# interactiveaudiolab/ppgs

Hardware: AMD Instinct MI355X
Metric: PPG frames/sec (whole node), mel repr, batch=32x1000 frames (higher is better)
Workload: dtype bf16; 1 GPU; configs[1]: mel representation, batch=32 x 1000 frames per GPU, audio resident in HBM -> (32,40,1000) fp32 posteriors in HBM; batch=32, frames=1000, per_gpu_batches=1, parallelism=utterance-sharded x1, no data-path collective

## Files before the change

ppgs_amd/csrc/ppg_frontend.hip:

```cpp
#include "ppg_lds.h"
#include "ppg_launch.h"

#include <hip/hip_fp16.h>

namespace {

constexpr int NFFT = 1024;
constexpr int HOP = 160;
constexpr int NBINS = 513;
constexpr int NMELS = 80;
constexpr int PADR = (NFFT - HOP) / 2;
constexpr int FPB = ppg::kFrontendFrames;
constexpr int SEG = NFFT + (FPB - 1) * HOP;
constexpr int BUF = NFFT + NFFT / 16;
constexpr int MSEG = ppg::kMelSegment;
constexpr int NS = ppg::kMelSteps;
constexpr int MROW = 1088;
__device__ __forceinline__ int sigma(int c) { return (0x6c >> (2 * c)) & 3; }

constexpr int OFF_TW = 0;
constexpr int SEGP = (SEG + 255) / 256 * 256;
constexpr int OFF_SEG = OFF_TW + 64 * 8;
constexpr int OFF_FFT = OFF_SEG + 2 * SEGP * 4;
constexpr int OFF_MAG = OFF_FFT + 4 * BUF * 8;
constexpr int LDS_BYTES = OFF_MAG + FPB * MROW;
constexpr int TEAMS = 2;
constexpr int CU_LDS_BYTES = 163840;
static_assert(2 * LDS_BYTES <= CU_LDS_BYTES && LDS_BYTES % 16 == 0, "two teams per CU; a two-team workgroup = the CU's LDS");
static_assert(OFF_MAG % 16 == 0 && MROW % 16 == 0, "fragment reads are 16-byte aligned");

typedef float cplx __attribute__((ext_vector_type(2)));
__device__ __forceinline__ cplx cadd(cplx a, cplx b) { return a + b; }
__device__ __forceinline__ cplx csub(cplx a, cplx b) { return a - b; }
__device__ __forceinline__ cplx cadd_mi(cplx a, cplx b) {
    cplx r;
    asm("v_pk_add_f32 %0, %1, %2 op_sel:[1,0] op_sel_hi:[0,1] neg_hi:[1,0]" : "=v"(r) : "v"(b), "v"(a));
    return r;
}
__device__ __forceinline__ cplx csub_mi(cplx a, cplx b) {
    cplx r;
    asm("v_pk_add_f32 %0, %1, %2 op_sel:[1,0] op_sel_hi:[0,1] neg_lo:[1,0]" : "=v"(r) : "v"(b), "v"(a));
    return r;
}
__device__ __forceinline__ cplx cmul(cplx a, cplx w) {
    cplx t, r;
    asm("v_pk_mul_f32 %0, %1, %2 op_sel:[0,0] op_sel_hi:[0,1]" : "=v"(t) : "v"(a), "v"(w));
    asm("v_fma_f32 %0, -%1, %2, %3" : "=v"(r.x) : "v"(a.y), "v"(w.y), "v"(t.x));
    asm("v_fma_f32 %0, %1, %2, %3" : "=v"(r.y) : "v"(a.y), "v"(w.x), "v"(t.y));
    return r;
}

template <bool CMI = false>
__device__ __forceinline__ void radix4(cplx& A, cplx& B, cplx& C, cplx& D) {
    const cplx apc = CMI ? cadd_mi(A, C) : cadd(A, C), amc = CMI ? csub_mi(A, C) : csub(A, C);
    const cplx bpd = cadd(B, D), bmd = csub(B, D);
    A = cadd(apc, bpd);
    B = cadd_mi(amc, bmd);
    C = csub(apc, bpd);
    D = csub_mi(amc, bmd);
}

template <int M>
__device__ __forceinline__ cplx w16() {
    constexpr float c1 = 0.92387953251128674f, s1 = 0.38268343236508977f, r = 0.70710678118654752f;
    if constexpr (M == 1) return cplx{c1, -s1};
    else if constexpr (M == 2) return cplx{r, -r};
    else if constexpr (M == 3) return cplx{s1, -c1};
    else if constexpr (M == 6) return cplx{-r, -r};
    else { static_assert(M == 9, "exponent"); return cplx{-c1, s1}; }
}

__device__ __forceinline__ void dft16(cplx (&x)[16]) {
#pragma unroll
    for (int r = 0; r < 4; ++r) radix4(x[r], x[r + 4], x[r + 8], x[r + 12]);
    x[5] = cmul(x[5], w16<1>());  x[9] = cmul(x[9], w16<2>());   x[13] = cmul(x[13], w16<3>());
    x[6] = cmul(x[6], w16<2>());   x[14] = cmul(x[14], w16<6>());
    x[7] = cmul(x[7], w16<3>());  x[11] = cmul(x[11], w16<6>()); x[15] = cmul(x[15], w16<9>());
    radix4(x[0], x[1], x[2], x[3]);
    radix4(x[4], x[5], x[6], x[7]);
    radix4<true>(x[8], x[9], x[10], x[11]);
    radix4(x[12], x[13], x[14], x[15]);
    cplx t;
#define PPG_SWAP(a, b) t = x[a]; x[a] = x[b]; x[b] = t;
    PPG_SWAP(1, 4) PPG_SWAP(2, 8) PPG_SWAP(3, 12) PPG_SWAP(6, 9) PPG_SWAP(7, 13) PPG_SWAP(11, 14)
#undef PPG_SWAP
}

__device__ __forceinline__ int pad(int i) { return i + (i >> 4); }

__device__ __forceinline__ void wave_sync() {
    asm volatile("s_waitcnt lgkmcnt(0)" ::: "memory");
    __builtin_amdgcn_fence(__ATOMIC_ACQ_REL, "wavefront");
    __builtin_amdgcn_wave_barrier();
}

template <bool SPEC, class SRC>
__device__ __forceinline__ void frontend_body(
    const ppg::FrontendTables& tb, const SRC& src, int total_groups, int wide_ok, __half* __restrict__ spec, __half* __restrict__ mel)
{
    extern __shared__ __attribute__((aligned(16))) char smem_all[];
    const int team = TEAMS == 1 ? 0 : __builtin_amdgcn_readfirstlane((int)(threadIdx.x >> 8));
    char* smem = smem_all + team * LDS_BYTES;
    cplx* tw = reinterpret_cast<cplx*>(smem + OFF_TW);
    float* seg0 = reinterpret_cast<float*>(smem + OFF_SEG);

    const int tid = threadIdx.x & 255;
    const int lane = tid & 63;
    const int wave = __builtin_amdgcn_readfirstlane(tid >> 6);
    cplx* buf = reinterpret_cast<cplx*>(smem + OFF_FFT) + wave * BUF;

    if (tid < 64) { const float2 w = tb.twiddle[16 * tid]; tw[tid] = cplx{w.x, w.y}; }
    reinterpret_cast<uint32_t*>(smem + OFF_MAG + (tid >> 4) * MROW + 1024)[tid & 15] = 0u;

    float hreg[16];
    cplx t1[16];
#pragma unroll
    for (int j = 0; j < 16; ++j) hreg[j] = tb.hann[lane + 64 * j];
#pragma unroll
    for (int k = 1; k < 16; ++k) { const float2 w = tb.twiddle[lane * k]; t1[k] = cplx{w.x, w.y}; }

    int step_frag[NS], step_off[NS], step_block[NS];
#pragma unroll
    for (int i = 0; i < NS; ++i) {
        const int4 e = tb.mel_prog[wave * NS + i];
        step_frag[i] = __builtin_amdgcn_readfirstlane(e.x);
        step_off[i] = __builtin_amdgcn_readfirstlane(e.y);
        step_block[i] = __builtin_amdgcn_readfirstlane(e.z);
    }

    auto stage = [&](int grp, int into) { src.stage(tb, grp, into, seg0, wave, lane, wide_ok); };
    const int stride = TEAMS * gridDim.x;
    const int first_group = TEAMS * blockIdx.x + team;
    if (first_group < total_groups) stage(first_group, 0);
    asm volatile("s_waitcnt vmcnt(0)" ::: "memory");

#ifdef PPG_FE_TIMING
    int stamp_group = 0;
    auto stamp = [&](int k) {
        if (tb.dbg && blockIdx.x == 0 && lane == 0 && stamp_group == 2) tb.dbg[wave * 16 + k] = __builtin_amdgcn_s_memtime();
    };
#else
    auto stamp = [&](int) {};
#endif
    int half = 0;
    const int trips = (total_groups - TEAMS * (int)blockIdx.x + stride - 1) / stride;
    int grp = first_group;
    for (int trip = 0; trip < trips; ++trip, grp += stride, half ^= 1) {
        const bool active = grp < total_groups;
        int b, f0, frames;
        src.group(grp, active, b, f0, frames);
        const float* seg = seg0 + half * SEGP;
        int pitch = src.pitch(frames);
        asm volatile("" : "+s"(pitch));
#ifdef PPG_FE_TIMING
        ++stamp_group;
#endif
        stamp(0);
        __syncthreads();
        stamp(1);

        auto transform = [&](const int j, const bool verify = false) {
            const int fa = f0 + 2 * j;
            if (fa >= frames) return;
            cplx x[16];
            {
                const float* sa = seg + (2 * j) * HOP + lane;
#pragma unroll
                for (int i = 0; i < 16; ++i) {
                    x[i] = cplx{sa[64 * i], sa[64 * i + HOP]} * hreg[i];
                }
                dft16(x);
#pragma unroll
                for (int k = 1; k < 16; ++k) x[k] = cmul(x[k], t1[k]);
#pragma unroll
                for (int k = 0; k < 16; ++k) buf[17 * lane + k] = x[k];
            }
            wave_sync();
            const int p0 = lane + (lane >> 4);
            {
#pragma unroll
                for (int i = 0; i < 16; ++i) x[i] = buf[p0 + 68 * i];
                dft16(x);
                const int p = lane >> 4, q = lane & 15;
#pragma unroll
                for (int k = 1; k < 16; ++k) x[k] = cmul(x[k], tw[p * k]);
                cplx* dst = buf + q + 272 * p;
#pragma unroll
                for (int k = 0; k < 16; ++k) dst[17 * k] = x[k];
            }
            wave_sync();
#pragma unroll
            for (int m = 0; m < 4; ++m) {
                cplx* z = buf + p0 + 68 * m;
                cplx A = z[0], B = z[272], C = z[544], D = z[816];
                radix4(A, B, C, D);
                z[0] = A; z[272] = B; z[544] = C; z[816] = D;
            }
            wave_sync();
            const int nb = (NFFT - lane) + ((NFFT - lane) >> 4);
            const int odd = lane & 1;
            const int row = j + 8 * odd;
            char* wdst = smem + OFF_MAG + row * MROW + ((((lane >> 3) ^ sigma(row >> 2)) << 2) + ((lane >> 1) & 3)) * 4;
            const uint32_t sel = odd ? 0x07060302u : 0x01000504u;
            auto split_bin = [&](int r, __half& ha, __half& hb) {
                const int k = lane + 64 * r;
                const cplx zk = buf[p0 + 68 * r];
                const cplx zn = buf[(r == 0 && lane == 0) ? 0 : nb - 68 * r];
                const float ar = 0.5f * (zk.x + zn.x), ai = 0.5f * (zk.y - zn.y);
                const float br = 0.5f * (zk.y + zn.y), bi = -0.5f * (zk.x - zn.x);
                ha = __float2half_rn(__builtin_amdgcn_sqrtf(ar * ar + ai * ai + 1e-6f));
                hb = __float2half_rn(__builtin_amdgcn_sqrtf(br * br + bi * bi + 1e-6f));
                if constexpr (SPEC) {
                    if (verify) return;
                    spec[(uint32_t)(b * NBINS + k) * (uint32_t)pitch + (uint32_t)fa] = ha;
                    if (fa + 1 < frames) spec[(uint32_t)(b * NBINS + k) * (uint32_t)pitch + (uint32_t)fa + 1u] = hb;
                }
            };
#pragma unroll
            for (int r = 0; r < 8; ++r) {
                __half ha, hb;
                split_bin(r, ha, hb);
                const uint32_t pk = (uint32_t)__half_as_ushort(ha) | ((uint32_t)__half_as_ushort(hb) << 16);
                const uint32_t other = (uint32_t)__builtin_amdgcn_mov_dpp((int)pk, 0xB1, 0xf, 0xf, true);
                const uint32_t val = __builtin_amdgcn_perm(pk, other, sel);
                *reinterpret_cast<uint32_t*>(wdst + 128 * r) = val;
            }
            if (verify) return;
            if (lane == 0) {
                __half ha, hb;
                split_bin(8, ha, hb);
                *reinterpret_cast<uint32_t*>(smem + OFF_MAG + j * MROW + ((64 ^ sigma(j >> 2)) << 4)) = __half_as_ushort(ha);
                *reinterpret_cast<uint32_t*>(smem + OFF_MAG + (j + 8) * MROW + ((64 ^ sigma((j + 8) >> 2)) << 4)) = __half_as_ushort(hb);
            }
        };

        transform(wave);
        stamp(2);
        if (!(wide_ok & 4) && grp + stride < total_groups) stage(grp + stride, half ^ 1);
        stamp(3);
        transform(wave + 4);
        stamp(4);
        u32x4 whi[NS], wlo[NS];
        asm volatile("s_waitcnt vmcnt(0)" ::: "memory");
        if (mel) {
            uint32_t loff = lane * 16;
            asm volatile("" : "+v"(loff));
#pragma unroll
            for (int i = 0; i < NS; ++i) {
                const char* src = reinterpret_cast<const char*>(tb.mel_img) + (size_t)step_frag[i] * 1024;
                whi[i] = *reinterpret_cast<const u32x4*>(src + loff);
                wlo[i] = *reinterpret_cast<const u32x4*>(src + 1024 + loff);
            }
        }
        __syncthreads();
        stamp(5);
        if (mel) {
            const int n = lane & 15, g = lane >> 4;
            const char* brow = smem + OFF_MAG + n * MROW + ((g ^ sigma(n >> 2)) << 4);
            f32x4 acc = {0.f, 0.f, 0.f, 0.f};
            const int frame = f0 + (n < 8 ? 2 * n : 2 * (n - 8) + 1);
#pragma unroll
            for (int i = 0; i < NS; ++i) {
                const u32x4 bfi = *reinterpret_cast<const u32x4*>(brow + step_off[i]);
                PrecF16::mma(acc, whi[i], bfi);
                PrecF16::mma(acc, wlo[i], bfi);
                const int block = step_block[i];
                if ((i == MSEG - 1 || i == NS - 1) && block >= 0) {
                    if (frame < frames) {
#pragma unroll
                        for (int e = 0; e < 4; ++e) {
                            const int m = 16 * block + 4 * g + e;
                            mel[(uint32_t)(b * NMELS + m) * (uint32_t)pitch + (uint32_t)frame] =
                                __float2half_rn(logf(fmaxf(acc[e] * (1.0f / 65536.0f), 1e-5f)));
                        }
                    }
                    acc = f32x4{0.f, 0.f, 0.f, 0.f};
                }
            }
        }
        stamp(6);
        if (wide_ok & 4) {
            __syncthreads();
            if (grp + stride < total_groups) stage(grp + stride, half ^ 1);
            asm volatile("s_waitcnt vmcnt(0)" ::: "memory");
        }
        if constexpr (SRC::kCarry) { if (active) src.carry_forward(grp, tid); }
    }
}

struct BatchSource {
    static constexpr bool kCarry = false;
    const float* __restrict__ audio;
    int samples, frames, groups_per_row;
    __device__ __forceinline__ void group(int grp, bool active, int& b, int& f0, int& nframes) const {
        b = active ? grp / groups_per_row : 0;
        f0 = active ? (grp - b * groups_per_row) * FPB : frames;
        nframes = frames;
    }
    __device__ __forceinline__ int pitch(int nframes) const { return nframes; }
    __device__ __forceinline__ void stage(const ppg::FrontendTables& tb, int grp, int into, float* seg0, int wave, int lane, int wide_ok) const {
        const int b = grp / groups_per_row;
        const int f0 = (grp - b * groups_per_row) * FPB;
        const float* arow = audio + (size_t)b * samples;
        const uint32_t dst = lds_addr(seg0) + into * (SEGP * 4);
        const int first = f0 * HOP - PADR;
        if ((wide_ok & 1) && first >= 0 && first + SEGP <= samples) {
#pragma unroll
            for (int j = 0; j < (SEGP / 256 + 3) / 4; ++j) {
                const int piece = wave + 4 * j;
                if (piece >= SEGP / 256) break;
                glds16_saddr(reinterpret_cast<const char*>(arow + first), (uint32_t)(piece * 1024 + lane * 16), dst + piece * 1024);
            }
            return;
        }
#pragma unroll 2
        for (int piece = wave; piece < SEGP / 64; piece += 4) {
            int src = first + piece * 64 + lane;
            if (src < 0) src = -src;
            if (src >= samples) src = 2 * (samples - 1) - src;
            const float* p = (src >= 0 && src < samples) ? arow + src : tb.hann;
            asm volatile("s_mov_b32 m0, %1\n\ts_nop 0\n\tglobal_load_lds_dword %0, off"
                         :: "v"(p), "s"(__builtin_amdgcn_readfirstlane(dst + piece * 256)) : "memory", "m0");
        }
    }
};

template <bool SPEC>
__global__ __launch_bounds__(256 * TEAMS, 2 / TEAMS) void frontend_kernel(
    ppg::FrontendTables tb, const float* __restrict__ audio, int samples, int frames,
    int groups_per_row, int total_groups, int wide_ok, __half* __restrict__ spec, __half* __restrict__ mel)
{
    frontend_body<SPEC>(tb, BatchSource{audio, samples, frames, groups_per_row}, total_groups, wide_ok, spec, mel);
}

struct StreamSource {
    static constexpr bool kCarry = true;
    ppg::FrontendStreamArgs a;
    __device__ __forceinline__ void group(int grp, bool active, int& b, int& f0, int& nframes) const {
        const int l = active ? grp / a.groups_per_item : 0;
        nframes = active ? a.item[l].frames : 0;
        f0 = active ? (grp - l * a.groups_per_item) * FPB : 0;
        b = a.item0 + l;
    }
    __device__ __forceinline__ int pitch(int) const { return a.out_pitch; }
    __device__ __forceinline__ const float* sample(const ppg::FrontendStreamItem& it, int l, int pos) const {
        return pos < it.split ? a.carry + ((size_t)(2 * (a.item0 + l) + it.cur) * a.cap + (pos - it.cbase))
                              : a.chunk + ((size_t)(a.item0 + l) * a.chunk_pitch + (pos - it.split));
    }
    __device__ __forceinline__ void stage(const ppg::FrontendTables& tb, int grp, int into, float* seg0, int wave, int lane, int) const {
        const int l = grp / a.groups_per_item;
        const int f0 = (grp - l * a.groups_per_item) * FPB;
        const ppg::FrontendStreamItem it = a.item[l];
        if (f0 >= it.frames) return;
        const uint32_t dst = lds_addr(seg0) + into * (SEGP * 4);
        const int first = f0 * HOP - PADR;
#pragma unroll 2
        for (int piece = wave; piece < SEGP / 64; piece += 4) {
            int pos = first + piece * 64 + lane;
            if (pos < it.lo) pos = 2 * it.lo - pos;
            if (pos >= it.hi) pos = 2 * (it.hi - 1) - pos;
            const float* p = (pos >= it.cbase && pos < it.hi) ? sample(it, l, pos) : tb.hann;
            asm volatile("s_mov_b32 m0, %1\n\ts_nop 0\n\tglobal_load_lds_dword %0, off"
                         :: "v"(p), "s"(__builtin_amdgcn_readfirstlane(dst + piece * 256)) : "memory", "m0");
        }
    }
    __device__ __forceinline__ void carry_forward(int grp, int tid) const {
        const int l = grp / a.groups_per_item;
        if (grp != l * a.groups_per_item) return;
        const ppg::FrontendStreamItem it = a.item[l];
        float* next = a.carry + (size_t)(2 * (a.item0 + l) + (it.cur ^ 1)) * a.cap;
        for (int pos = it.keep + tid; pos < it.hi; pos += 256) next[pos - it.keep] = *sample(it, l, pos);
    }
};

__global__ __launch_bounds__(256 * TEAMS, 2 / TEAMS) void frontend_stream_kernel(
    ppg::FrontendTables tb, StreamSource src, int total_groups, __half* __restrict__ mel)
{
    frontend_body<false>(tb, src, total_groups, 0, nullptr, mel);
}

}

namespace ppg {

hipError_t launch_frontend(const FrontendTables& tb, const float* audio, int batch, int samples,
                           void* spec, void* mel, hipStream_t s) {
    const int frames = samples / HOP;
    const int groups_per_row = (frames + FPB - 1) / FPB;
    if (mel && (!tb.mel_img || !tb.mel_prog)) return hipErrorInvalidValue;
    if ((double)batch * NBINS * frames >= 4294967296.0) return hipErrorInvalidValue;
    const int total = groups_per_row * batch;
    static LdsLimit limit[2];
    const void* kernel = spec ? reinterpret_cast<const void*>(frontend_kernel<true>) : reinterpret_cast<const void*>(frontend_kernel<false>);
    const hipError_t e = limit[spec != nullptr].ensure(kernel, CU_LDS_BYTES);
    if (e != hipSuccess) return e;
    static int slots = 0;
    if (slots == 0) {
        int dev = 0, cus = 0;
        if (hipGetDevice(&dev) != hipSuccess ||
            hipDeviceGetAttribute(&cus, hipDeviceAttributeMultiprocessorCount, dev) != hipSuccess || cus <= 0)
            cus = 256;
        slots = 2 * cus;
    }
    const int rounds = (total + slots - 1) / slots;
    const int teams = (total + rounds - 1) / rounds;
    const int grid = (teams + TEAMS - 1) / TEAMS;
    int wide_ok = (reinterpret_cast<uintptr_t>(audio) % 16 == 0 && samples % 4 == 0) ? 1 : 0;
    size_t lds_bytes = TEAMS == 2 ? CU_LDS_BYTES : LDS_BYTES;
    static const int fe_debug = env_experiment("PPGS_AMD_FE_DEBUG", 0);
    if (fe_debug & 1) wide_ok = 0;
    if (fe_debug & 4) wide_ok |= 4;
    if (fe_debug & 16) lds_bytes = TEAMS * LDS_BYTES;
    if (spec)
        hipLaunchKernelGGL(frontend_kernel<true>, dim3(grid), dim3(256 * TEAMS), lds_bytes, s, tb, audio, samples, frames,
                           groups_per_row, total, wide_ok, reinterpret_cast<__half*>(spec), reinterpret_cast<__half*>(mel));
    else
        hipLaunchKernelGGL(frontend_kernel<false>, dim3(grid), dim3(256 * TEAMS), lds_bytes, s, tb, audio, samples, frames,
                           groups_per_row, total, wide_ok, reinterpret_cast<__half*>(spec), reinterpret_cast<__half*>(mel));
    return hipGetLastError();
}

hipError_t launch_frontend_stream(const FrontendTables& tb, const FrontendStreamArgs& args, int items, void* mel, hipStream_t s) {
    if (!tb.mel_img || !tb.mel_prog || items <= 0 || items > kFrontendStreamItems || args.groups_per_item <= 0)
        return hipErrorInvalidValue;
    if ((double)(args.item0 + items) * NMELS * args.out_pitch >= 4294967296.0) return hipErrorInvalidValue;
    static LdsLimit limit;
    const hipError_t e = limit.ensure(reinterpret_cast<const void*>(frontend_stream_kernel), CU_LDS_BYTES);
    if (e != hipSuccess) return e;
    static int slots = 0;
    if (slots == 0) {
        int dev = 0, cus = 0;
        if (hipGetDevice(&dev) != hipSuccess ||
            hipDeviceGetAttribute(&cus, hipDeviceAttributeMultiprocessorCount, dev) != hipSuccess || cus <= 0)
            cus = 256;
        slots = 2 * cus;
    }
    const int total = args.groups_per_item * items;
    const int rounds = (total + slots - 1) / slots;
    const int teams = (total + rounds - 1) / rounds;
    const int grid = (teams + TEAMS - 1) / TEAMS;
    hipLaunchKernelGGL(frontend_stream_kernel, dim3(grid), dim3(256 * TEAMS), CU_LDS_BYTES, s, tb, StreamSource{args}, total,
                       reinterpret_cast<__half*>(mel));
    return hipGetLastError();
}

}
```

Before: 48.01 million frames/s.

## Fuse final radix-4 FFT stage into real-split magnitude pass in registers

Removes the separate last radix-4 pass that wrote back to LDS, along with its wave_sync. Each lane now fetches both a bin and its mirror column, runs the radix-4 butterflies in registers, and computes the two-real-FFT split and magnitudes directly. This saves one LDS round trip and one barrier per FFT. In exchange, each lane holds more registers, descending bins are written with scattered 16-bit LDS stores, and the verify early-return path is dropped.

```diff
diff --git a/ppgs_amd/csrc/ppg_frontend.hip b/ppgs_amd/csrc/ppg_frontend.hip
--- a/ppgs_amd/csrc/ppg_frontend.hip
+++ b/ppgs_amd/csrc/ppg_frontend.hip
@@ -189,48 +189,63 @@
                 for (int k = 0; k < 16; ++k) dst[17 * k] = x[k];
             }
             wave_sync();
-#pragma unroll
-            for (int m = 0; m < 4; ++m) {
-                cplx* z = buf + p0 + 68 * m;
-                cplx A = z[0], B = z[272], C = z[544], D = z[816];
-                radix4(A, B, C, D);
-                z[0] = A; z[272] = B; z[544] = C; z[816] = D;
-            }
-            wave_sync();
-            const int nb = (NFFT - lane) + ((NFFT - lane) >> 4);
             const int odd = lane & 1;
             const int row = j + 8 * odd;
             char* wdst = smem + OFF_MAG + row * MROW + ((((lane >> 3) ^ sigma(row >> 2)) << 2) + ((lane >> 1) & 3)) * 4;
             const uint32_t sel = odd ? 0x07060302u : 0x01000504u;
-            auto split_bin = [&](int r, __half& ha, __half& hb) {
-                const int k = lane + 64 * r;
-                const cplx zk = buf[p0 + 68 * r];
-                const cplx zn = buf[(r == 0 && lane == 0) ? 0 : nb - 68 * r];
+            char* mag = smem + OFF_MAG + j * MROW;
+            const int sa = sigma(j >> 2);
+            auto split_bin = [&](int k, cplx zk, cplx zn, __half& ha, __half& hb) {
                 const float ar = 0.5f * (zk.x + zn.x), ai = 0.5f * (zk.y - zn.y);
                 const float br = 0.5f * (zk.y + zn.y), bi = -0.5f * (zk.x - zn.x);
                 ha = __float2half_rn(__builtin_amdgcn_sqrtf(ar * ar + ai * ai + 1e-6f));
                 hb = __float2half_rn(__builtin_amdgcn_sqrtf(br * br + bi * bi + 1e-6f));
                 if constexpr (SPEC) {
-                    if (verify) return;
                     spec[(uint32_t)(b * NBINS + k) * (uint32_t)pitch + (uint32_t)fa] = ha;
                     if (fa + 1 < frames) spec[(uint32_t)(b * NBINS + k) * (uint32_t)pitch + (uint32_t)fa + 1u] = hb;
                 }
             };
-#pragma unroll
-            for (int r = 0; r < 8; ++r) {
+            auto ascending = [&](int r, cplx zk, cplx zn) {
                 __half ha, hb;
-                split_bin(r, ha, hb);
+                split_bin(lane + 64 * r, zk, zn, ha, hb);
                 const uint32_t pk = (uint32_t)__half_as_ushort(ha) | ((uint32_t)__half_as_ushort(hb) << 16);
                 const uint32_t other = (uint32_t)__builtin_amdgcn_mov_dpp((int)pk, 0xB1, 0xf, 0xf, true);
                 const uint32_t val = __builtin_amdgcn_perm(pk, other, sel);
                 *reinterpret_cast<uint32_t*>(wdst + 128 * r) = val;
-            }
-            if (verify) return;
+            };
+            auto descending = [&](int k, cplx zk, cplx zn) {
+                __half ha, hb;
+                split_bin(k, zk, zn, ha, hb);
+                const int o = (((k >> 3) ^ sa) << 4) + ((k & 7) << 1);
+                *reinterpret_cast<__half*>(mag + o) = ha;
+                *reinterpret_cast<__half*>(mag + 8 * MROW + (o ^ 32)) = hb;
+            };
+            auto fetch = [&](int r, int q2, cplx (&a)[4], cplx (&m)[4]) {
+                const cplx* c1 = buf + p0 + 68 * r;
+                const cplx* c2 = buf + pad(q2);
+#pragma unroll
+                for (int i = 0; i < 4; ++i) { a[i] = c1[272 * i]; m[i] = c2[272 * i]; }
+            };
+            auto finish = [&](int r, int q2, cplx (&a)[4], cplx (&m)[4], const bool self) {
+                radix4(a[0], a[1], a[2], a[3]);
+                radix4(m[0], m[1], m[2], m[3]);
+                ascending(r, a[0], self ? a[0] : m[3]);
+                ascending(r + 4, a[1], self ? a[3] : m[2]);
+                descending(q2, m[0], self ? m[3] : a[3]);
+                descending(q2 + 256, m[1], self ? m[2] : a[2]);
+            };
+            const int qa = lane == 0 ? 128 : 256 - lane, qb = 192 - lane;
+            cplx a[4], am[4], c[4], cm[4];
+            fetch(0, qa, a, am);
+            fetch(1, qb, c, cm);
+            finish(0, qa, a, am, lane == 0);
+            finish(1, qb, c, cm, false);
             if (lane == 0) {
+                const cplx z512 = a[2];
                 __half ha, hb;
-                split_bin(8, ha, hb);
-                *reinterpret_cast<uint32_t*>(smem + OFF_MAG + j * MROW + ((64 ^ sigma(j >> 2)) << 4)) = __half_as_ushort(ha);
-                *reinterpret_cast<uint32_t*>(smem + OFF_MAG + (j + 8) * MROW + ((64 ^ sigma((j + 8) >> 2)) << 4)) = __half_as_ushort(hb);
+                split_bin(512, z512, z512, ha, hb);
+                *reinterpret_cast<uint32_t*>(mag + ((64 ^ sa) << 4)) = __half_as_ushort(ha);
+                *reinterpret_cast<uint32_t*>(mag + 8 * MROW + ((64 ^ sa ^ 2) << 4)) = __half_as_ushort(hb);
             }
         };
 
```

Measured after the change: 48.33 million frames/s, median of 6. No clear change (+0.7%).
